# Vanlightly/vsr-tlaplus

Hardware: NVIDIA H100
Metric: unique states explored/sec (VSR.tla, shipped VSR.cfg constants) (higher is better)
Workload: dtype u32

## Files before the change

### vsr-tlaplus_b200/csrc/vsr_gpu.cu

```cuda
#include <stddef.h>
#include <stdio.h>
#include <stdlib.h>
#include <string.h>

#include <algorithm>
#include <chrono>
#include <string>
#include <vector>

#include "vsr_engine.h"

namespace vsr {

const GpuOps* find_gpu_ops(int R, int V, int K) {
#define X(r, v, k) \
    if (R == r && V == v && K == k) return GpuThunks<Layout<r, v, k>>::get();
    VSR_FOR_EACH_CONFIG(X)
#undef X
    return nullptr;
}

}

using namespace vsr;
// ... 247 lines not shown

int vsr_engine_expand(VsrEngine* e) { return vsr_engine_step(e, 0, e->n_cur, 0, nullptr, nullptr); }

int vsr_engine_insert_records(VsrEngine* e, const void* dev_records, uint64_t n) {
    if (!e->level_open) {
        int rc = engine_reset_level(e);
        if (rc) return rc;
    }
    if (n == 0) return 0;
    InsertParams q;
    fill_params(e, q.e);
    q.recs = (const uint8_t*)dev_records;
    q.n = n;
    CK(cudaEventRecord(e->ev0, e->stream));
    CK(e->g->launch_insert(q, e->stream));
    CK(cudaEventRecord(e->ev1, e->stream));
    e->st.kernel_launches++;
    CK(cudaEventSynchronize(e->ev1));
    float ms = 0;
    cudaEventElapsedTime(&ms, e->ev0, e->ev1);
    e->level_ms_acc += ms;
    e->level_ms_insert_acc += ms;
    return 0;
}

int vsr_engine_finish_level(VsrEngine* e, VsrLevelInfo* out) {
    DevCounters c;
    CK(cudaMemcpyAsync(&c, e->ctr, sizeof c, cudaMemcpyDeviceToHost, e->stream));
    e->st.bytes_d2h += sizeof c;
    CK(cudaStreamSynchronize(e->stream));
    const uint64_t fcap_total = e->frontier_cap + e->frontier_host_cap;
    if (c.tie_count > 0 && c.tie_count <= e->tie_cap && !c.overflow && c.out_count <= fcap_total) {
        const size_t tb = (size_t)e->g->tie_bytes;
        std::vector<uint8_t> host(c.tie_count * tb);
        CK(cudaMemcpyAsync(host.data(), e->ties, host.size(), cudaMemcpyDeviceToHost, e->stream));
        CK(cudaStreamSynchronize(e->stream));
        std::vector<const uint8_t*> recs;
        for (uint64_t i = 0; i < c.tie_count; i++) recs.push_back(host.data() + i * tb);
        auto key = [](const uint8_t* r) { return (const TieRec*)r; };
        std::sort(recs.begin(), recs.end(), [&](const uint8_t* a, const uint8_t* b) {
            const TieRec *x = key(a), *y = key(b);
            if (x->fp != y->fp) return x->fp < y->fp;
            if (x->check != y->check) return x->check < y->check;
            if (x->auxkey != y->auxkey) return x->auxkey < y->auxkey;
            if (x->parent != y->parent) return x->parent < y->parent;
            return x->cand < y->cand;
        });
        std::vector<uint8_t> best;
        uint64_t nbest = 0;
        for (size_t i = 0; i < recs.size(); i++) {
            if (i && key(recs[i])->fp == key(recs[i - 1])->fp && key(recs[i])->check == key(recs[i - 1])->check) continue;
            best.insert(best.end(), recs[i], recs[i] + tb);
            nbest++;
        }
        CK(cudaMemcpyAsync(e->ties, best.data(), best.size(), cudaMemcpyHostToDevice, e->stream));
        static const unsigned long long ones = ~0ull;
        CK(cudaMemcpyAsync(&e->ctr->viol_id, &ones, 8, cudaMemcpyHostToDevice, e->stream));
        CK(cudaMemsetAsync(&e->ctr->viol_which, 0, sizeof(int), e->stream));
        ExpandParams p;
        fill_params(e, p);
        CK(e->g->launch_patch(p, e->ties, nbest, c.out_count, e->stream));
        e->st.kernel_launches++;
        CK(cudaMemcpyAsync(&c, e->ctr, sizeof c, cudaMemcpyDeviceToHost, e->stream));
        CK(cudaStreamSynchronize(e->stream));
        e->st.bytes_d2h += host.size() + sizeof c;
        e->st.bytes_h2d += best.size();
    }
    VsrLevelInfo li;
    memset(&li, 0, sizeof li);
    li.new_states = c.out_count;
    li.generated = c.generated;
    li.frontier_in = e->n_cur;
    li.ties = c.ties;
    li.collisions = c.collisions;
    li.violation = c.viol_id != ~0ull;
    li.violation_id = c.viol_id;
    li.violation_mask = c.viol_which;
    li.deadlock = c.dead_id != ~0ull;
    li.deadlock_id = c.dead_id;
    li.error_code = c.error;
    li.overflow = c.overflow;
    li.ms = e->level_ms_acc;
    li.ms_insert = e->level_ms_insert_acc;
    if (c.overflow) {
        snprintf(e->last_error, sizeof e->last_error, "capacity exceeded (%s): %llu new states this level, frontier capacity %llu",
                 c.overflow == 1 ? "frontier" : (c.overflow == 2 ? "tie list" : (c.overflow == 3 ? "send buffer" : "seen-set")), (unsigned long long)c.out_count,
                 (unsigned long long)fcap_total);
    }
    if (!li.overflow && e->st.distinct + c.out_count > e->table_cap - e->table_cap / 8) {
        li.overflow = 4;
        snprintf(e->last_error, sizeof e->last_error, "capacity exceeded (seen-set): %llu distinct states in %llu slots",
                 (unsigned long long)(e->st.distinct + c.out_count), (unsigned long long)e->table_cap);
    }
    const uint64_t n_new = c.out_count <= fcap_total ? c.out_count : fcap_total;
    e->st.generated += c.generated;
    e->st.distinct += n_new;
    e->st.h2_ties += c.ties;
    e->st.fp_collisions += c.collisions;
    e->st.probe_total += c.probes;
    e->st.seconds_kernels += e->level_ms_acc * 1e-3;
    if (c.error && !e->st.error_code) e->st.error_code = c.error;
    const int gen_level = e->level + 1;
    if (e->level >= 1 && e->level - 1 < VSR_MAX_LEVELS) {
        e->st.level_generated[e->level - 1] = c.generated;
        e->st.level_ms[e->level - 1] = e->level_ms_acc;
        e->st.levels_expanded = e->level;
    }
    if (n_new > 0 && gen_level - 1 < VSR_MAX_LEVELS) {
        e->st.level_sizes[gen_level - 1] = n_new;
        e->st.num_levels = gen_level;
    }
    if (li.violation && e->st.violation_level == 0) {
        e->st.violation_level = gen_level;
        e->st.violation_id = c.viol_id;
    }
    e->cur ^= 1;
    e->cur_base = e->next_base;
    e->n_cur = n_new;
    e->next_base += n_new;
    e->level = gen_level;
    e->level_open = false;
    if (e->opts.collect_levels) {
        std::vector<uint8_t> host((size_t)n_new * e->g->bytes);
        if (n_new && vsr_engine_read_frontier(e, 0, n_new, host.data())) return VSR_RC_SYSTEM;
        e->collected.push_back(std::move(host));
    }
    if (out) *out = li;
    return 0;
}

uint64_t vsr_engine_frontier_size(const VsrEngine* e) { return e->n_cur; }

int vsr_engine_read_frontier(VsrEngine* e, uint64_t first, uint64_t n, void* host_out) {
    if (first + n > e->n_cur) return VSR_RC_ERROR;
    const uint64_t S = (uint64_t)e->g->bytes;
    const uint64_t in_dev = first < e->frontier_cap ? std::min(n, e->frontier_cap - first) : 0;
    if (in_dev) CK(cudaMemcpy(host_out, (const uint8_t*)e->frontier[e->cur] + first * S, in_dev * S, cudaMemcpyDeviceToHost));
    if (n > in_dev) memcpy((uint8_t*)host_out + in_dev * S, (const uint8_t*)e->frontier_host[e->cur] + (first + in_dev - e->frontier_cap) * S, (n - in_dev) * S);
    return 0;
}

int vsr_engine_trace_record(VsrEngine* e, uint64_t local_id, uint64_t* parent_out, uint32_t* cand_out) {
    if (!e->trace || local_id >= e->trace_cap) return VSR_RC_ERROR;
    uint64_t t = 0;
    CK(cudaMemcpy(&t, e->trace + local_id, 8, cudaMemcpyDeviceToHost));
    e->st.bytes_d2h += 8;
    *parent_out = (t >> 12) & GID_MASK;
    *cand_out = (uint32_t)(t & 0xFFF);
    return 0;
}

int vsr_engine_lookup(VsrEngine* e, const void* state, int* level_out, int* owner_out) {
    const ModelOps* ops = e->m->ops;
    uint64_t fp = ops->fingerprint((const uint32_t*)state, e->m->run.use_view);
    if (fp == 0) fp = 1;
    const int owner = e->world > 1 ? owner_of(fp, e->owner_shift) : e->rank;
    if (owner_out) *owner_out = owner;
    *level_out = 0;
    if (owner != e->rank) return 0;
    const uint32_t chk = e->g->check_hash((const uint32_t*)state, e->m->run.use_view);
    unsigned long long* d = (unsigned long long*)&e->ctr->work_next;
    lookup_kernel<<<1, 1, 0, e->stream>>>(e->table, e->table_cap, fp, chk, d);
    CK(cudaGetLastError());
    unsigned long long meta = 0;
    CK(cudaMemcpyAsync(&meta, d, 8, cudaMemcpyDeviceToHost, e->stream));
    CK(cudaStreamSynchronize(e->stream));
// ... 237 lines not shown
```

### vsr-tlaplus_b200/csrc/vsr_gpu.cuh

```cuda
#ifndef VSR_GPU_CUH
#define VSR_GPU_CUH

#include <cuda_runtime.h>
#include <stdint.h>

#include "vsr_actions.h"

namespace vsr {

struct DevCounters {
    unsigned long long out_count;
    unsigned long long generated;
    unsigned long long ties;
    unsigned long long collisions;
    unsigned long long probes;
    unsigned long long viol_id;
    unsigned long long dead_id;
    unsigned long long tie_count;
    int error;
    int overflow;
    int viol_which;
    int _pad;
    unsigned long long work_next;
    unsigned long long drain_next;
    unsigned int send_count[8];
};

struct TieRec {
    uint64_t fp;
    uint64_t parent;
    uint32_t auxkey, cand, check, _pad;
};

struct RecHdr {
    uint64_t fp;
    uint64_t tm;
};
constexpr int MAX_WORLD = 8;


struct ExpandParams {
    const uint32_t* in;
    unsigned long long n_in;
    unsigned long long in_base;
    const uint32_t* in_hi;
    unsigned long long in_split;
    uint32_t* out;
    uint32_t* out_hi;
    unsigned long long out_split;
    unsigned long long out_cap;
    unsigned long long out_base;
    uint64_t* table;
    unsigned long long table_cap;
    uint64_t* trace;
    unsigned long long trace_cap;
    DevCounters* ctr;
    uint8_t* ties;
    unsigned long long tie_cap;
    const uint64_t* fp_tab;
    RunCfg run;
    int level;
    int check_deadlock;
    int rank, world, owner_shift;
    uint8_t* push[MAX_WORLD];
    unsigned long long push_cap;
    int push_direct;
    const uint8_t* drain[MAX_WORLD];
    unsigned int drain_n[MAX_WORLD];
    unsigned long long drain_total;
};

struct InsertParams {
    const uint8_t* recs;
    unsigned long long n;
    ExpandParams e;
};


__device__ __forceinline__ void cas128(uint64_t* p, uint64_t s0, uint64_t s1, uint64_t& o0, uint64_t& o1) {
    asm volatile(
        "{\n\t.reg .b128 cmp, swp, old;\n\tmov.b128 cmp, {%2, %3};\n\tmov.b128 swp, {%4, %5};\n\t"
        "atom.global.relaxed.gpu.cas.b128 old, [%6], cmp, swp;\n\tmov.b128 {%0, %1}, old;\n\t}"
        : "=l"(o0), "=l"(o1)
        : "l"(0ull), "l"(0ull), "l"(s0), "l"(s1), "l"(p)
        : "memory");
}
__device__ __forceinline__ void ld128_cg(const uint64_t* p, uint64_t& a, uint64_t& b) {
    asm volatile("ld.global.cg.v2.u64 {%0, %1}, [%2];" : "=l"(a), "=l"(b) : "l"(p) : "memory");
}
__device__ __forceinline__ uint64_t mix64(uint64_t x) {
    x ^= x >> 30; x *= 0xbf58476d1ce4e5b9ULL;
    x ^= x >> 27; x *= 0x94d049bb133111ebULL;
    x ^= x >> 31;
    return x;
}
template <class L, bool USE_VIEW, class W> VSR_HD uint32_t check_hash_t(const W& w) {
    constexpr int full = L::VIEW_BITS >> 5, rem = L::VIEW_BITS & 31;
    constexpr int nw = USE_VIEW ? (full + (rem ? 1 : 0)) : L::NW;
    uint32_t h = 0x9747b28cu;
VSR_UNROLL
    for (int i = 0; i < nw; i++) {
        uint32_t k = rdw(w, i);
        if (USE_VIEW && i == full) k &= (1u << rem) - 1u;
        h ^= k;
        h = ((h << 13) | (h >> 19)) * 5u + 0xe6546b64u;
    }
    h ^= h >> 16; h *= 0x85ebca6bu; h ^= h >> 13; h *= 0xc2b2ae35u; h ^= h >> 16;
    return h;
}
// ... 8 lines not shown
__host__ __device__ __forceinline__ uint64_t make_trec(uint64_t parent_gid, uint32_t cand) { return (parent_gid << 12) | (cand & 0xFFFu); }

__device__ __forceinline__ uint64_t make_meta(int level, uint32_t auxkey, uint32_t check) {
    return ((uint64_t)(uint32_t)level << 56) | ((uint64_t)(auxkey & 0xFFFFFFu) << 32) | check;
}

#ifndef VSR_BUCKET
#define VSR_BUCKET 2
#endif
struct Probe { uint64_t e[2 * VSR_BUCKET]; };
__device__ __forceinline__ void ld256_cg(const uint64_t* p, uint64_t& a, uint64_t& b, uint64_t& c, uint64_t& d) {
    asm volatile("ld.global.cg.v2.u64 {%0, %1}, [%4];\n\tld.global.cg.v2.u64 {%2, %3}, [%4+16];"
                 : "=l"(a), "=l"(b), "=l"(c), "=l"(d) : "l"(p) : "memory");
}
__device__ __forceinline__ unsigned long long table_home(unsigned long long cap, uint64_t fp) {
    return __umul64hi(fp * 0x9E3779B97F4A7C15ULL, cap / VSR_BUCKET) * VSR_BUCKET;
}
__device__ __forceinline__ void probe_load(const uint64_t* table, unsigned long long h, Probe& p) {
#if VSR_BUCKET == 1
    ld128_cg(table + 2 * h, p.e[0], p.e[1]);
#elif VSR_BUCKET == 2
    ld128_cg(table + 2 * h, p.e[0], p.e[1]);
#elif VSR_BUCKET == 4
    ld256_cg(table + 2 * h, p.e[0], p.e[1], p.e[2], p.e[3]);
    ld256_cg(table + 2 * h + 4, p.e[4], p.e[5], p.e[6], p.e[7]);
#else
#error "VSR_BUCKET must be 1, 2 or 4"
#endif
}
__device__ __forceinline__ int table_insert_from(uint64_t* table, unsigned long long cap, unsigned long long h, Probe p, uint64_t fp, uint64_t meta,
                                                 unsigned& probes, unsigned& collisions) {
    for (unsigned tries = 0;; tries++) {
        if (tries > (1u << 16)) return INS_FULL;
        probes++;
VSR_UNROLL
        for (int j = 0; j < VSR_BUCKET; j++) {
            uint64_t e0, e1;
            if (VSR_BUCKET == 2 && j == 1) {
                ld128_cg(table + 2 * (h + 1), e0, e1);
            } else {
                e0 = p.e[2 * j];
                e1 = p.e[2 * j + 1];
            }
            if (e0 == 0) {
                cas128(table + 2 * (h + j), fp, meta, e0, e1);
                if (e0 == 0 && e1 == 0) return INS_NEW;
            }
            for (int again = 0; e1 == 0 && again < 64; again++) ld128_cg(table + 2 * (h + j), e0, e1);
            if (e0 == fp) {
                if ((uint32_t)e1 == (uint32_t)meta) {
                    const bool same_level = (e1 >> 56) == (meta >> 56);
                    const bool same_aux = ((e1 >> 32) & 0xFFFFFF) == ((meta >> 32) & 0xFFFFFF);
                    return (same_level && !same_aux) ? INS_TIE : INS_DUP;
                }
                collisions++;
            }
        }
        h += VSR_BUCKET;
        if (h >= cap) h = 0;
        probe_load(table, h, p);
    }
}
__device__ __forceinline__ int table_insert(uint64_t* table, unsigned long long cap, uint64_t fp, uint64_t meta,
                                            unsigned& probes, unsigned& collisions) {
    const unsigned long long h = table_home(cap, fp);
    Probe p;
    probe_load(table, h, p);
    return table_insert_from(table, cap, h, p, fp, meta, probes, collisions);
}

__device__ __forceinline__ void bulk_store(void* gdst, const void* ssrc, uint32_t bytes) {
    asm volatile("fence.proxy.async.shared::cta;" ::: "memory");
    const uint32_t s = (uint32_t)__cvta_generic_to_shared(ssrc);
    asm volatile("cp.async.bulk.global.shared::cta.bulk_group [%0], [%1], %2;" ::"l"(gdst), "r"(s), "r"(bytes) : "memory");
    asm volatile("cp.async.bulk.commit_group;" ::: "memory");
    asm volatile("cp.async.bulk.wait_group.read 0;" ::: "memory");
}

template <int NW> __device__ __forceinline__ uint32_t* out_state(const ExpandParams& P, unsigned long long i) {
    return i < P.out_split ? P.out + i * NW : P.out_hi + (i - P.out_split) * NW;
}


constexpr int SCAP = 64;
#ifdef VSR_QPS
constexpr int QPS = VSR_QPS;
#else
constexpr int QPS = 10;
#endif

template <class L> struct WarpStage {
    alignas(16) uint32_t stage[SCAP * L::NW + 32];
    unsigned long long tstage[SCAP];
    int sn;
};
template <class L, int WARPS> struct BlockSmemT {
    static constexpr int NS = WARPS * 32;
    static constexpr int NG = 13;
    uint64_t fp_tab[8 * 256];
    uint32_t par[NS * (L::NW + 1)];
    static constexpr int QCAP = QPS * NS;
    uint16_t pool[QCAP];
    int qcount[NG];
    int take;
    unsigned long long round_first;
    WarpStage<L> w[WARPS];
};
template <class L> struct ExpandCfg {
    static constexpr size_t SMEM_ONE = 227 * 1024 - 512, SMEM_TWO = 113 * 1024;
    static constexpr int max_grp() { int m = 0; for (int g = 0; g < Ops<L>::NGRP; g++) m = Ops<L>::grp_size(g) > m ? Ops<L>::grp_size(g) : m; return m; }
    template <int W> static constexpr int pick_one() {
        if constexpr (W < 18) return 0;
        else if constexpr (sizeof(BlockSmemT<L, W>) <= SMEM_ONE) return W;
        else return pick_one<W - 2>();
    }
    static constexpr int W2 = sizeof(BlockSmemT<L, 16>) <= SMEM_TWO ? 16 : (sizeof(BlockSmemT<L, 12>) <= SMEM_TWO ? 12 : 8);
    static constexpr int W1 = max_grp() < 64 ? pick_one<32>() : 0;
#ifdef VSR_FORCE_WARPS
    static constexpr int WARPS = VSR_FORCE_WARPS;
#else
    static constexpr int WARPS = W1 >= 2 * W2 - 4 ? W1 : W2;
#endif
    static constexpr int BLOCKS = WARPS > 16 ? 1 : 2;
    typedef BlockSmemT<L, WARPS> Smem;
};

template <class L, bool MULTI> struct Expander {
    typedef Ops<L> O_;
    typedef typename ExpandCfg<L>::Smem Smem;
    static constexpr int WARPS = ExpandCfg<L>::WARPS, NS = Smem::NS;
    const ExpandParams& P;
    Smem& B;
    WarpStage<L>& S;
    const int lane, warp, tid;
    const uint32_t* mine = nullptr;
    bool have = false;

    __device__ Expander(const ExpandParams& p, Smem& b) : P(p), B(b), S(b.w[threadIdx.x >> 5]), lane(threadIdx.x & 31), warp(threadIdx.x >> 5), tid(threadIdx.x) {}

    static __device__ __noinline__ void flush(const ExpandParams& P, WarpStage<L>& S, int lane, int n) {
        const int sn = S.sn;
        unsigned long long base = 0;
        if (lane == 0) base = atomicAdd(&P.ctr->out_count, (unsigned long long)n);
        base = __shfl_sync(0xffffffffu, base, 0);
        if (lane < n) {
            const unsigned long long t = S.tstage[lane];
            if (t >> 63) {
                atomicMin(&P.ctr->viol_id, P.out_base + base + lane);
                S.tstage[lane] = t & ~(1ull << 63);
            }
        }
        __syncwarp();
        if (base + n > P.out_cap) {
            if (lane == 0) atomicExch(&P.ctr->overflow, 1);
        } else {
            if (lane == 0) {
                if (base + n <= P.out_split) bulk_store(P.out + base * L::NW, S.stage, (uint32_t)(n * L::BYTES));
                else if (base >= P.out_split) bulk_store(P.out_hi + (base - P.out_split) * L::NW, S.stage, (uint32_t)(n * L::BYTES));
                else {
                    const int n1 = (int)(P.out_split - base);
                    bulk_store(P.out + base * L::NW, S.stage, (uint32_t)(n1 * L::BYTES));
                    bulk_store(P.out_hi, S.stage + n1 * L::NW, (uint32_t)((n - n1) * L::BYTES));
                }
            }
            if (P.trace && lane < n && P.out_base + base + lane < P.trace_cap) P.trace[P.out_base + base + lane] = S.tstage[lane];
        }
        __syncwarp();
        const int rest = sn - n;
        for (int i0 = 0; i0 < rest * L::NW; i0 += 32) {
            const int i = i0 + lane;
            uint32_t v = 0;
            if (i < rest * L::NW) v = S.stage[n * L::NW + i];
            __syncwarp();
            if (i < rest * L::NW) S.stage[i] = v;
        }
        unsigned long long t = 0;
        if (lane < rest) t = S.tstage[n + lane];
        __syncwarp();
        if (lane < rest) S.tstage[lane] = t;
        if (lane == 0) S.sn = rest;
        __syncwarp();
    }

    typedef uint32_t* Row;
    static constexpr int gcd32(int a) { int g = 32; while (a % g) g >>= 1; return g; }
    static constexpr int SKEW_P = 32 / gcd32(L::NW);
    static __device__ __forceinline__ Row scratch(WarpStage<L>& S, int lane) { return &S.stage[(32 + lane) * L::NW + lane / SKEW_P]; }

    static __device__ __forceinline__ void push_records(const ExpandParams& P, WarpStage<L>& S, int lane, const RegRow<L::NW>& v, int send_to, uint64_t fp,
                                                        uint64_t tm) {
        const unsigned senders = __ballot_sync(0xffffffffu, send_to >= 0);
        if (!senders) return;
        constexpr int RB = L::BYTES + (int)sizeof(RecHdr), RW = RB / 4;
        constexpr int CAPREC = (32 * L::BYTES) / RB;
        static_assert(CAPREC >= 16, "two passes must cover a batch");
        int off = 0, cnt = 0, rnk = 0;
        unsigned mymask = 0;
        for (int d = 0; d < P.world; d++) {
            const unsigned m = __ballot_sync(0xffffffffu, send_to == d);
            if (send_to > d) off += __popc(m);
            if (send_to == d) { mymask = m; cnt = __popc(m); rnk = __popc(m & ((1u << lane) - 1u)); }
        }
        unsigned base = 0;
        if (send_to >= 0 && rnk == 0) base = atomicAdd(&P.ctr->send_count[send_to], (unsigned)cnt);
        base = __shfl_sync(0xffffffffu, base, mymask ? __ffs(mymask) - 1 : 0);
        const bool fits = send_to >= 0 && (unsigned long long)base + (unsigned)cnt <= P.push_cap;
        if (send_to >= 0 && !fits && rnk == 0) atomicExch(&P.ctr->overflow, 3);
        if (P.push_direct) {
            if (fits) {
                uint4* d = reinterpret_cast<uint4*>(P.push[send_to] + (size_t)(base + (unsigned)rnk) * RB);
                VSR_UNROLL
                for (int q = 0; q < L::NW / 4; q++) d[q] = make_uint4(v.w[4 * q], v.w[4 * q + 1], v.w[4 * q + 2], v.w[4 * q + 3]);
                d[L::NW / 4] = make_uint4((uint32_t)fp, (uint32_t)(fp >> 32), (uint32_t)tm, (uint32_t)(tm >> 32));
            }
            return;
        }
        const int pos = off + rnk, total = __popc(senders);
        uint32_t* sbuf = &S.stage[32 * L::NW];
        for (int lo = 0; lo < total; lo += CAPREC) {
            const int hi = lo + CAPREC < total ? lo + CAPREC : total;
            if (send_to >= 0 && pos >= lo && pos < hi) {
                uint32_t* r = sbuf + (pos - lo) * RW;
                VSR_UNROLL
                for (int j = 0; j < L::NW; j++) r[j] = v.w[j];
                r[L::NW] = (uint32_t)fp; r[L::NW + 1] = (uint32_t)(fp >> 32);
                r[L::NW + 2] = (uint32_t)tm; r[L::NW + 3] = (uint32_t)(tm >> 32);
            }
            __syncwarp();
            if (fits) {
                const int st = off > lo ? off : lo, en = off + cnt < hi ? off + cnt : hi;
                if (pos == st && st < en)
                    bulk_store(P.push[send_to] + (size_t)(base + (unsigned)(st - off)) * RB, sbuf + (st - lo) * RW, (uint32_t)((en - st) * RB));
            }
            __syncwarp();
        }
    }

    static __device__ __forceinline__ unsigned long long commit(const ExpandParams& P, WarpStage<L>& S, int lane, const RegRow<L::NW>& v, bool live, uint64_t fp,
                                                                uint32_t chk, uint32_t auxkey, unsigned long long home, const Probe& first, unsigned long long trec,
                                                                unsigned mult, bool check_inv = true) {
        unsigned gen = 0, probes = 0, coll = 0;
        int sn = S.sn;
        bool isnew = false;
        int bad = 0;
        if (live) {
            const uint64_t meta = make_meta(P.level, auxkey, chk);
            gen = mult;
            const int r = table_insert_from(P.table, P.table_cap, home, first, fp, meta, probes, coll);
            isnew = r == INS_NEW;
            if (r == INS_FULL) atomicExch(&P.ctr->overflow, 4);
            if (isnew && check_inv) bad = O_::invariant(P.run, v);
            if (coll) atomicAdd(&P.ctr->collisions, (unsigned long long)coll);
            if (r == INS_TIE) {
                atomicAdd(&P.ctr->ties, 1ull);
                const unsigned long long t = atomicAdd(&P.ctr->tie_count, 1ull);
                if (t < P.tie_cap) {
                    TieRec rec;
                    rec.fp = fp; rec.parent = trec >> 12; rec.auxkey = auxkey; rec.cand = (uint32_t)(trec & 0xFFFu); rec.check = chk; rec._pad = 0;
                    uint8_t* dst = P.ties + t * (sizeof(TieRec) + L::BYTES);
                    *(TieRec*)dst = rec;
                    VSR_UNROLL
                    for (int j = 0; j < L::NW; j++) ((uint32_t*)(dst + sizeof(TieRec)))[j] = v.w[j];
                } else atomicExch(&P.ctr->overflow, 2);
            }
        }
        const unsigned newmask = __ballot_sync(0xffffffffu, isnew);
        __syncwarp();
        if (isnew) {
            const int slot = sn + __popc(newmask & ((1u << lane) - 1u));
            VSR_UNROLL
            for (int j = 0; j < L::NW; j++) S.stage[slot * L::NW + j] = v.w[j];
            if (bad) {
                trec |= 1ull << 63;
                atomicOr(&P.ctr->viol_which, bad);
            }
            S.tstage[slot] = trec;
        }
        sn += __popc(newmask);
        __syncwarp();
        if (lane == 0) S.sn = sn;
        __syncwarp();
        while (sn >= 32) {
            flush(P, S, lane, 32);
            sn -= 32;
        }
        return (unsigned long long)gen | ((unsigned long long)probes << 32);
    }

    static __device__ __noinline__ unsigned long long emit(const ExpandParams& P, Smem& B, WarpStage<L>& S, int lane, const Row n, int mult,
                                                           int cand, int si, bool act, bool check_inv) {
        int send_to = -1;
        uint64_t fp = 0;
        uint32_t chk = 0, auxkey = 0;
        unsigned long long home = 0, trec = 0;
        Probe first = {};
        bool live = false;
        RegRow<L::NW> v;
        if (act && mult > 0) {
            VSR_UNROLL
            for (int j = 0; j < L::NW; j++) v.w[j] = rdw(n, j);
        }
        if (act) {
            if (mult < 0) {
                atomicCAS(&P.ctr->error, 0, mult);
            } else if (mult > 0) {
                fp = fp64_view8<L>(B.fp_tab, v, P.run.use_view != 0);
                if (fp == 0) fp = 1;
                const int owner = MULTI ? owner_of(fp, P.owner_shift) : P.rank;
                trec = make_trec(make_gid(P.rank, P.in_base + B.round_first + si), (uint32_t)cand);
                if (owner == P.rank) {
                    live = true;
                    home = table_home(P.table_cap, fp);
                    probe_load(P.table, home, first);
                    chk = check_hash<L>(v, P.run.use_view != 0);
                    auxkey = O_::aux_key(v);
                } else {
                    send_to = owner;
                }
            }
        }
        if (MULTI) {
            __syncwarp();
            push_records(P, S, lane, v, send_to, fp, trec | ((uint64_t)(unsigned)mult << 56));
        }
        return commit(P, S, lane, v, live, fp, chk, auxkey, home, first, trec, (unsigned)mult, check_inv);
    }

    struct DrainPre {
        uint64_t fp, tm;
        unsigned long long home;
        Probe first;
        const uint4* rec;
        bool have;
    };
    unsigned long long dchunk = ~0ull;
    __device__ __forceinline__ unsigned long long drain_chunks() const { return (P.drain_total + 31) / 32; }
    __device__ __forceinline__ unsigned long long drain_claim() {
        unsigned long long c = 0;
        if (lane == 0) c = atomicAdd(&P.ctr->drain_next, 1ull);
        return c;
    }
    __device__ __forceinline__ DrainPre drain_begin(unsigned long long chunk) {
        constexpr int RB = L::BYTES + (int)sizeof(RecHdr);
        DrainPre d;
        unsigned long long i = chunk * 32 + lane;
        d.have = chunk < drain_chunks() && i < P.drain_total;
        d.fp = d.tm = 0;
        d.home = 0;
        d.first = Probe{};
        d.rec = nullptr;
        if (d.have) {
            int s = 0;
            while (s < P.world - 1 && i >= P.drain_n[s]) { i -= P.drain_n[s]; s++; }
            d.rec = reinterpret_cast<const uint4*>(P.drain[s] + i * RB);
            const uint4 h = __ldcs(d.rec + L::NW / 4);
            d.fp = ((uint64_t)h.y << 32) | h.x;
            d.tm = ((uint64_t)h.w << 32) | h.z;
            d.home = table_home(P.table_cap, d.fp);
            probe_load(P.table, d.home, d.first);
        }
        return d;
    }
    __device__ __forceinline__ void drain_end(const DrainPre& d) {
        RegRow<L::NW> v;
        uint32_t chk = 0, auxkey = 0;
        if (d.have) {
            VSR_UNROLL
            for (int q = 0; q < L::NW / 4; q++) {
                const uint4 x = __ldcs(d.rec + q);
                v.w[4 * q] = x.x; v.w[4 * q + 1] = x.y; v.w[4 * q + 2] = x.z; v.w[4 * q + 3] = x.w;
            }
            chk = check_hash<L>(v, P.run.use_view != 0);
            auxkey = O_::aux_key(v);
        }
        tally(commit(P, S, lane, v, d.have, d.fp, chk, auxkey, d.home, d.first, d.tm & ((1ull << 56) - 1ull), (unsigned)((d.tm >> 56) & 0xFu)));
    }
    __device__ void drain() {
        const unsigned long long nchunks = drain_chunks();
        if (dchunk == ~0ull) dchunk = __shfl_sync(0xffffffffu, drain_claim(), 0);
        while (dchunk < nchunks) {
            const unsigned long long nx = drain_claim();
            const DrainPre d = drain_begin(dchunk);
            drain_end(d);
            dchunk = __shfl_sync(0xffffffffu, nx, 0);
        }
    }

    static constexpr int NG = O_::NGRP;
    static __host__ __device__ constexpr int moff(int g) { int o = 0; for (int h = 0; h < g; h++) o += O_::grp_words(h); return o; }
    static constexpr int MW = moff(NG);
    static constexpr int PW = (NG + 1) / 2;
    static __host__ __device__ constexpr int max_grp() { int m = 0; for (int g = 0; g < NG; g++) m = O_::grp_size(g) > m ? O_::grp_size(g) : m; return m; }
    static constexpr int TBITS = NS <= 512 ? 9 : 10;
    static_assert(NS <= (1 << TBITS) && max_grp() < (1 << (16 - TBITS)), "pool item does not fit 16 bits");
    static_assert(max_grp() * NS < 65536, "16-bit packed counters");

    template <int G> __device__ __forceinline__ void guards(const RegRow<L::NW>& st, uint32_t* m, uint32_t* pc) {
        O_::template enabled_group<G>(P.run, st, m + moff(G));
        uint32_t c = 0;
        VSR_UNROLL
        for (int k = 0; k < O_::grp_words(G); k++) c += (uint32_t)__popc(m[moff(G) + k]);
        pc[G >> 1] += c << (16 * (G & 1));
        if constexpr (G + 1 < NG) guards<G + 1>(st, m, pc);
    }
    template <int G, bool FAST> __device__ __forceinline__ void push(uint32_t* m, const uint32_t* ex, const uint32_t* wb, int st) {
        int pos = st + (int)((wb[G >> 1] >> (16 * (G & 1))) & 0xFFFFu) + (int)((ex[G >> 1] >> (16 * (G & 1))) & 0xFFFFu);
        VSR_UNROLL
        for (int k = 0; k < O_::grp_words(G); k++) {
            uint32_t mm = m[moff(G) + k], left = 0;
            while (mm) {
                const int bit = __ffs(mm) - 1;
                mm &= mm - 1;
                if (FAST || pos < Smem::QCAP) B.pool[pos] = (uint16_t)(tid | ((k * 32 + bit) << TBITS));
                else left |= 1u << bit;
                pos++;
            }
            if (!FAST) m[moff(G) + k] = left;
        }
        if constexpr (G + 1 < NG) {
            const int nst = FAST ? st + B.qcount[G] : (st + B.qcount[G] < Smem::QCAP ? st + B.qcount[G] : Smem::QCAP);
            push<G + 1, FAST>(m, ex, wb, nst);
        }
    }
    template <int G> __device__ __forceinline__ void leftovers(uint32_t* m) {
        VSR_UNROLL
        for (int k = 0; k < O_::grp_words(G); k++) {
            while (__any_sync(0xffffffffu, m[moff(G) + k] != 0)) {
                const bool inl = m[moff(G) + k] != 0;
                int cand = 0;
                if (inl) {
                    const int bit = __ffs(m[moff(G) + k]) - 1;
                    m[moff(G) + k] &= m[moff(G) + k] - 1;
                    cand = O_::grp_begin(G) + k * 32 + bit;
                }
                tally(apply<G>(P, B, S, lane, mine, cand, tid, inl));
            }
        }
        if constexpr (G + 1 < NG) leftovers<G + 1>(m);
    }
    __device__ __forceinline__ void scan_all() {
        uint32_t m[MW], pc[PW];
        VSR_UNROLL
        for (int i = 0; i < MW; i++) m[i] = 0;
        VSR_UNROLL
        for (int i = 0; i < PW; i++) pc[i] = 0;
        if (have) {
            RegRow<L::NW> st;
            VSR_UNROLL
            for (int i = 0; i < L::NW; i++) st.w[i] = mine[i];
            guards<0>(st, m, pc);
        }
        uint32_t ex[PW], wb[PW];
        VSR_UNROLL
        for (int i = 0; i < PW; i++) ex[i] = pc[i];
        VSR_UNROLL
        for (int o = 1; o < 32; o <<= 1) {
            VSR_UNROLL
            for (int i = 0; i < PW; i++) {
                const uint32_t t = __shfl_up_sync(0xffffffffu, ex[i], o);
                if (lane >= o) ex[i] += t;
            }
        }
        uint32_t mytot = 0, anyc = 0;
        VSR_UNROLL
        for (int g = 0; g < NG; g++) {
            const uint32_t t = (__shfl_sync(0xffffffffu, ex[g >> 1], 31) >> (16 * (g & 1))) & 0xFFFFu;
            if (lane == g) mytot = t;
        }
        VSR_UNROLL
        for (int i = 0; i < PW; i++) { anyc |= pc[i]; ex[i] -= pc[i]; }
        uint32_t mybase = 0;
        if (lane < NG && mytot) mybase = (uint32_t)atomicAdd(&B.qcount[lane], (int)mytot);
        VSR_UNROLL
        for (int i = 0; i < PW; i++) wb[i] = 0;
        VSR_UNROLL
        for (int g = 0; g < NG; g++) wb[g >> 1] |= (__shfl_sync(0xffffffffu, mybase, g) & 0xFFFFu) << (16 * (g & 1));
        if (P.check_deadlock && have && !anyc) atomicMin(&P.ctr->dead_id, P.in_base + B.round_first + tid);
        __syncthreads();
#ifndef VSR_EXP_NO_PUSHFAST
        int all = 0;
        VSR_UNROLL
        for (int g = 0; g < NG; g++) all += B.qcount[g];
        if (all <= Smem::QCAP) {
            push<0, true>(m, ex, wb, 0);
            return;
        }
#endif
        push<0, false>(m, ex, wb, 0);
        uint32_t rest = 0;
        VSR_UNROLL
        for (int i = 0; i < MW; i++) rest |= m[i];
        if (__any_sync(0xffffffffu, rest != 0)) leftovers<0>(m);
    }
    template <int G> static __device__ __noinline__ unsigned long long apply(const ExpandParams& P, Smem& B, WarpStage<L>& S, int lane,
                                                                             const uint32_t* parent, int cand, int si, bool act) {
        const Row n = scratch(S, lane);
        int mult = 0;
        if (act) mult = O_::template step_grp<true, G>(P.run, parent, cand, n);
#ifdef VSR_EXP_INVSKIP
        return emit(P, B, S, lane, n, mult, cand, si, act, O_::may_falsify(G));
#else
        return emit(P, B, S, lane, n, mult, cand, si, act, true);
#endif
    }
    template <int G> static __device__ __forceinline__ unsigned long long batch(const ExpandParams& P, Smem& B, WarpStage<L>& S, int lane, int b,
                                                                                int k) {
        const bool act = lane < k;
        int cand = 0, si = 0;
        if (act) {
            const unsigned item = B.pool[b + lane];
            si = item & ((1 << TBITS) - 1);
            cand = O_::grp_begin(G) + (int)(item >> TBITS);
        }
        return apply<G>(P, B, S, lane, &B.par[si * (L::NW + 1)], cand, si, act);
    }
    unsigned long long acc_gen = 0, acc_probes = 0;
    __device__ __forceinline__ void tally(unsigned long long r) {
        acc_gen += (unsigned)r;
        acc_probes += r >> 32;
    }

    __device__ void run_round(unsigned long long first, int count) {
        const uint32_t* src = P.in + first * L::NW;
        if (first + count <= P.in_split) {
            for (int i = tid; i < count * L::NW; i += NS) B.par[(i / L::NW) * (L::NW + 1) + (i % L::NW)] = __ldg(src + i);
        } else {
            for (int i = tid; i < count * L::NW; i += NS) {
                const unsigned long long st = first + i / L::NW;
                const uint32_t* row = st < P.in_split ? P.in + st * L::NW : P.in_hi + (st - P.in_split) * L::NW;
                B.par[(i / L::NW) * (L::NW + 1) + (i % L::NW)] = __ldg(row + i % L::NW);
            }
        }
        if (tid < Smem::NG) B.qcount[tid] = 0;
        if (tid == 0) { B.round_first = first; B.take = 0; }
        __syncthreads();
        have = tid < count;
        mine = &B.par[(have ? tid : 0) * (L::NW + 1)];
        scan_all();
        __syncthreads();
        const int q = lane < Smem::NG ? B.qcount[lane] : 0;
        int inc = q;
        VSR_UNROLL
        for (int o = 1; o < 32; o <<= 1) {
            const int t = __shfl_up_sync(0xffffffffu, inc, o);
            if (lane >= o) inc += t;
        }
        const int seg_st = inc - q < Smem::QCAP ? inc - q : Smem::QCAP, seg_en = inc < Smem::QCAP ? inc : Smem::QCAP;
        const int nb = (seg_en - seg_st + 31) >> 5;
        int binc = nb;
        VSR_UNROLL
        for (int o = 1; o < 32; o <<= 1) {
            const int t = __shfl_up_sync(0xffffffffu, binc, o);
            if (lane >= o) binc += t;
        }
        const int total = __shfl_sync(0xffffffffu, binc, 31);
        for (;;) {
            int t = 0;
            if (lane == 0) t = atomicAdd(&B.take, 1);
            t = __shfl_sync(0xffffffffu, t, 0);
            if (t >= total) break;
            const int g = __popc(__ballot_sync(0xffffffffu, lane < Smem::NG && binc <= t));
            const int st = __shfl_sync(0xffffffffu, seg_st, g), en = __shfl_sync(0xffffffffu, seg_en, g);
            const int b = st + (t - __shfl_sync(0xffffffffu, binc - nb, g)) * 32;
            const int k = en - b < 32 ? en - b : 32;
            unsigned long long r;
            switch (g) {
            case 0: r = batch<0>(P, B, S, lane, b, k); break;   case 1: r = batch<1>(P, B, S, lane, b, k); break;
            case 2: r = batch<2>(P, B, S, lane, b, k); break;   case 3: r = batch<3>(P, B, S, lane, b, k); break;
            case 4: r = batch<4>(P, B, S, lane, b, k); break;   case 5: r = batch<5>(P, B, S, lane, b, k); break;
            case 6: r = batch<6>(P, B, S, lane, b, k); break;   case 7: r = batch<7>(P, B, S, lane, b, k); break;
            case 8: r = batch<8>(P, B, S, lane, b, k); break;   case 9: r = batch<9>(P, B, S, lane, b, k); break;
            case 10: r = batch<10>(P, B, S, lane, b, k); break; case 11: r = batch<11>(P, B, S, lane, b, k); break;
            default: r = batch<12>(P, B, S, lane, b, k); break;
            }
            tally(r);
        }
    }

    __device__ void finish() {
        while (S.sn > 0) flush(P, S, lane, S.sn < 32 ? S.sn : 32);
        for (int o = 16; o; o >>= 1) {
            acc_gen += __shfl_xor_sync(0xffffffffu, acc_gen, o);
            acc_probes += __shfl_xor_sync(0xffffffffu, acc_probes, o);
        }
        if (lane == 0) {
            atomicAdd(&P.ctr->generated, acc_gen);
            atomicAdd(&P.ctr->probes, acc_probes);
        }
    }
};

template <class L, bool MULTI> __global__ void __launch_bounds__(ExpandCfg<L>::WARPS * 32, ExpandCfg<L>::BLOCKS) expand_kernel(const __grid_constant__ ExpandParams P) {
    extern __shared__ __align__(128) unsigned char smem_raw[];
    typedef typename ExpandCfg<L>::Smem Smem;
    Smem& B = *reinterpret_cast<Smem*>(smem_raw);
    for (int i = threadIdx.x; i < 8 * 256; i += blockDim.x) B.fp_tab[i] = P.fp_tab[i];
    __shared__ unsigned long long next_round;
    Expander<L, MULTI> X(P, B);
    if ((threadIdx.x & 31) == 0) {
        WarpStage<L>& S = B.w[threadIdx.x >> 5];
        S.sn = 0;
    }
    const unsigned long long nrounds = (P.n_in + Smem::NS - 1) / Smem::NS;
    if (threadIdx.x == 0) next_round = atomicAdd(&P.ctr->work_next, 1ull);
    for (;;) {
        __syncthreads();
        const unsigned long long c = next_round;
        __syncthreads();
        if (c >= nrounds) break;
        if (threadIdx.x == 0) {
            next_round = atomicAdd(&P.ctr->work_next, 1ull);
            const unsigned long long nx = next_round;
            if (nx < nrounds && (nx + 1) * Smem::NS <= P.in_split) {
                const unsigned long long nfirst = nx * Smem::NS;
                const unsigned long long ncount = (P.n_in - nfirst) < (unsigned long long)Smem::NS ? (P.n_in - nfirst) : Smem::NS;
                asm volatile("cp.async.bulk.prefetch.L2.global [%0], %1;" ::"l"(P.in + nfirst * L::NW), "r"((uint32_t)(ncount * L::BYTES)) : "memory");
            }
        }
        const unsigned long long first = c * Smem::NS;
        const int count = (int)((P.n_in - first) < (unsigned long long)Smem::NS ? (P.n_in - first) : Smem::NS);
        X.run_round(first, count);
    }
    if (MULTI && P.drain_total) X.drain();
    X.finish();
}


template <class L> __global__ void __launch_bounds__(256) insert_kernel(const InsertParams Q) {
    const ExpandParams& P = Q.e;
    const unsigned long long i = (unsigned long long)blockIdx.x * blockDim.x + threadIdx.x;
    const int lane = threadIdx.x & 31;
    const bool have = i < Q.n;
    bool isnew = false;
    const uint8_t* rec = Q.recs + (have ? i : 0) * (L::BYTES + sizeof(RecHdr));
    const uint32_t* n = (const uint32_t*)rec;
    const RecHdr* h = (const RecHdr*)(rec + L::BYTES);
    unsigned probes = 0, coll = 0, nties = 0;
    unsigned long long gen = 0;
    uint64_t parent = 0;
    uint32_t cand = 0;
    if (have) {
        const uint64_t meta = make_meta(P.level, Ops<L>::aux_key(n), check_hash<L>(n, P.run.use_view != 0));
        const int r = table_insert(P.table, P.table_cap, h->fp, meta, probes, coll);
        isnew = r == INS_NEW;
        if (r == INS_FULL) atomicExch(&P.ctr->overflow, 4);
        gen = (h->tm >> 56) & 0xFu;
        parent = (h->tm >> 12) & ((1ull << 44) - 1ull);
        cand = (uint32_t)(h->tm & 0xFFFu);
        if (r == INS_TIE) {
            nties = 1;
            const unsigned long long t = atomicAdd(&P.ctr->tie_count, 1ull);
            if (t < P.tie_cap) {
                TieRec tr;
                tr.fp = h->fp; tr.parent = parent; tr.auxkey = (uint32_t)((meta >> 32) & 0xFFFFFF); tr.cand = cand;
                tr.check = (uint32_t)meta; tr._pad = 0;
                uint8_t* dst = P.ties + t * (sizeof(TieRec) + L::BYTES);
                *(TieRec*)dst = tr;
                for (int j = 0; j < L::NW; j++) ((uint32_t*)(dst + sizeof(TieRec)))[j] = n[j];
            } else atomicExch(&P.ctr->overflow, 2);
        }
    }
    for (int o = 16; o; o >>= 1) {
        gen += __shfl_xor_sync(0xffffffffu, gen, o);
        probes += __shfl_xor_sync(0xffffffffu, probes, o);
        coll += __shfl_xor_sync(0xffffffffu, coll, o);
        nties += __shfl_xor_sync(0xffffffffu, nties, o);
    }
    if (lane == 0) {
        if (gen) atomicAdd(&P.ctr->generated, gen);
        if (probes) atomicAdd(&P.ctr->probes, (unsigned long long)probes);
        if (coll) atomicAdd(&P.ctr->collisions, (unsigned long long)coll);
        if (nties) atomicAdd(&P.ctr->ties, (unsigned long long)nties);
    }
    const unsigned newmask = __ballot_sync(0xffffffffu, isnew);
    if (newmask) {
        unsigned long long base = 0;
        const int leader = __ffs(newmask) - 1;
        if (lane == leader) base = atomicAdd(&P.ctr->out_count, (unsigned long long)__popc(newmask));
        base = __shfl_sync(0xffffffffu, base, leader);
        if (isnew) {
            const unsigned long long pos = base + __popc(newmask & ((1u << lane) - 1u));
            if (pos < P.out_cap) {
                uint32_t* dst = out_state<L::NW>(P, pos);
                for (int j = 0; j < L::NW; j++) dst[j] = n[j];
                if (P.trace && P.out_base + pos < P.trace_cap) P.trace[P.out_base + pos] = make_trec(parent, cand);
                const int bad = Ops<L>::invariant(P.run, n);
                if (bad) {
                    atomicMin(&P.ctr->viol_id, P.out_base + pos);
                    atomicOr(&P.ctr->viol_which, bad);
                }
            } else atomicExch(&P.ctr->overflow, 1);
        }
    }
}

template <class L> __global__ void patch_ties_kernel(const ExpandParams P, const uint8_t* ties, unsigned long long ntie, unsigned long long n_out) {
    const unsigned long long i = (unsigned long long)blockIdx.x * blockDim.x + threadIdx.x;
    if (i >= n_out) return;
    uint32_t w[L::NW];
    uint32_t* st = out_state<L::NW>(P, i);
    for (int j = 0; j < L::NW; j++) w[j] = st[j];
    uint64_t fp = fp64_view8<L>(P.fp_tab, w, P.run.use_view != 0);
    if (fp == 0) fp = 1;
// ... 105 lines not shown
```

Before: 2.658 billion.

## Scan two frontier passes per round to halve block barriers per state

Each block round now covers PASSES×NS parent states. The scan phase runs once per pass, into separate queue-count and pool segments, and then a single batch phase drains both passes' candidate queues, amortising the round-end and scan barriers over twice the states. To fit in shared memory, the per-warp staging buffer shrinks to 32 rows when two passes are used, so commit flushes immediately instead of accumulating up to 64 rows. This means more global atomics on out_count and smaller bulk stores. Optional clock64 instrumentation behind a macro breaks round time into barrier, scan and batch components.

Result: faster. 2.963 billion (median of 6 runs) (+11.5%).

```diff
diff --git a/vsr-tlaplus_b200/csrc/vsr_gpu.cu b/vsr-tlaplus_b200/csrc/vsr_gpu.cu
--- a/vsr-tlaplus_b200/csrc/vsr_gpu.cu
+++ b/vsr-tlaplus_b200/csrc/vsr_gpu.cu
@@ -353,6 +353,15 @@
     li.overflow = c.overflow;
     li.ms = e->level_ms_acc;
     li.ms_insert = e->level_ms_insert_acc;
+#ifdef VSR_EXP_ROUNDCLK
+    {
+        double all = 0;
+        for (int i = 0; i < 5; i++) all += (double)c.roundclk[i];
+        if (all > 0)
+            fprintf(stderr, "roundclk rank %d depth %d  ms %.4f  warp-Gcycles %.4f  end_barrier %.4f  scan_barriers %.4f  batches %.4f  scan %.4f  other %.4f\n",
+                    e->rank, e->level, e->level_ms_acc, all * 1e-9, c.roundclk[0] / all, c.roundclk[1] / all, c.roundclk[2] / all, c.roundclk[3] / all, c.roundclk[4] / all);
+    }
+#endif
     if (c.overflow) {
         snprintf(e->last_error, sizeof e->last_error, "capacity exceeded (%s): %llu new states this level, frontier capacity %llu",
                  c.overflow == 1 ? "frontier" : (c.overflow == 2 ? "tie list" : (c.overflow == 3 ? "send buffer" : "seen-set")), (unsigned long long)c.out_count,
diff --git a/vsr-tlaplus_b200/csrc/vsr_gpu.cuh b/vsr-tlaplus_b200/csrc/vsr_gpu.cuh
--- a/vsr-tlaplus_b200/csrc/vsr_gpu.cuh
+++ b/vsr-tlaplus_b200/csrc/vsr_gpu.cuh
@@ -24,7 +24,13 @@
     unsigned long long work_next;
     unsigned long long drain_next;
     unsigned int send_count[8];
+#ifdef VSR_EXP_ROUNDCLK
+    unsigned long long roundclk[5];
+#endif
 };
+#ifdef VSR_EXP_ROUNDCLK
+enum { CLK_END = 0, CLK_SCANBAR = 1, CLK_BATCH = 2, CLK_SCAN = 3, CLK_OTHER = 4 };
+#endif
 
 struct TieRec {
     uint64_t fp;
@@ -199,39 +205,40 @@
 }
 
 
-constexpr int SCAP = 64;
 #ifdef VSR_QPS
 constexpr int QPS = VSR_QPS;
 #else
 constexpr int QPS = 10;
 #endif
 
-template <class L> struct WarpStage {
-    alignas(16) uint32_t stage[SCAP * L::NW + 32];
-    unsigned long long tstage[SCAP];
+template <class L, int ROWS> struct WarpStage {
+    alignas(16) uint32_t stage[ROWS * L::NW + 32];
+    unsigned long long tstage[ROWS];
     int sn;
 };
-template <class L, int WARPS> struct BlockSmemT {
+template <class L, int WARPS, int PASSES> struct BlockSmemT {
+    typedef WarpStage<L, PASSES == 2 ? 32 : 64> Stage;
     static constexpr int NS = WARPS * 32;
+    static constexpr int NR = PASSES * NS;
     static constexpr int NG = 13;
     uint64_t fp_tab[8 * 256];
-    uint32_t par[NS * (L::NW + 1)];
+    uint32_t par[NR * (L::NW + 1)];
     static constexpr int QCAP = QPS * NS;
-    uint16_t pool[QCAP];
-    int qcount[NG];
+    uint16_t pool[PASSES * QCAP];
+    int qcount[PASSES][NG];
     int take;
     unsigned long long round_first;
-    WarpStage<L> w[WARPS];
+    Stage w[WARPS];
 };
 template <class L> struct ExpandCfg {
     static constexpr size_t SMEM_ONE = 227 * 1024 - 512, SMEM_TWO = 113 * 1024;
     static constexpr int max_grp() { int m = 0; for (int g = 0; g < Ops<L>::NGRP; g++) m = Ops<L>::grp_size(g) > m ? Ops<L>::grp_size(g) : m; return m; }
     template <int W> static constexpr int pick_one() {
         if constexpr (W < 18) return 0;
-        else if constexpr (sizeof(BlockSmemT<L, W>) <= SMEM_ONE) return W;
+        else if constexpr (sizeof(BlockSmemT<L, W, 1>) <= SMEM_ONE) return W;
         else return pick_one<W - 2>();
     }
-    static constexpr int W2 = sizeof(BlockSmemT<L, 16>) <= SMEM_TWO ? 16 : (sizeof(BlockSmemT<L, 12>) <= SMEM_TWO ? 12 : 8);
+    static constexpr int W2 = sizeof(BlockSmemT<L, 16, 1>) <= SMEM_TWO ? 16 : (sizeof(BlockSmemT<L, 12, 1>) <= SMEM_TWO ? 12 : 8);
     static constexpr int W1 = max_grp() < 64 ? pick_one<32>() : 0;
 #ifdef VSR_FORCE_WARPS
     static constexpr int WARPS = VSR_FORCE_WARPS;
@@ -239,24 +246,49 @@
     static constexpr int WARPS = W1 >= 2 * W2 - 4 ? W1 : W2;
 #endif
     static constexpr int BLOCKS = WARPS > 16 ? 1 : 2;
-    typedef BlockSmemT<L, WARPS> Smem;
+#ifdef VSR_ROUND_PASSES
+    static constexpr int PASSES = VSR_ROUND_PASSES;
+#else
+    static constexpr int PASSES = BLOCKS == 1 && sizeof(BlockSmemT<L, WARPS, 2>) <= SMEM_ONE ? 2 : 1;
+#endif
+    typedef BlockSmemT<L, WARPS, PASSES> Smem;
 };
 
 template <class L, bool MULTI> struct Expander {
     typedef Ops<L> O_;
     typedef typename ExpandCfg<L>::Smem Smem;
-    static constexpr int WARPS = ExpandCfg<L>::WARPS, NS = Smem::NS;
+    typedef typename Smem::Stage Stage;
+    static constexpr int WARPS = ExpandCfg<L>::WARPS, NS = Smem::NS, PASSES = ExpandCfg<L>::PASSES;
+    static constexpr int SROWS = PASSES == 2 ? 32 : 64;
     const ExpandParams& P;
     Smem& B;
-    WarpStage<L>& S;
+    Stage& S;
     const int lane, warp, tid;
     const uint32_t* mine = nullptr;
     bool have = false;
-
-    __device__ Expander(const ExpandParams& p, Smem& b) : P(p), B(b), S(b.w[threadIdx.x >> 5]), lane(threadIdx.x & 31), warp(threadIdx.x >> 5), tid(threadIdx.x) {}
-
-    static __device__ __noinline__ void flush(const ExpandParams& P, WarpStage<L>& S, int lane, int n) {
-        const int sn = S.sn;
+    int pass = 0;
+    __device__ __forceinline__ int pass_i() const { return PASSES == 1 ? 0 : pass; }
+
+    __device__ Expander(const ExpandParams& p, Smem& b) : P(p), B(b), S(b.w[threadIdx.x >> 5]), lane(threadIdx.x & 31), warp(threadIdx.x >> 5), tid(threadIdx.x) {
+#ifdef VSR_EXP_ROUNDCLK
+        clk_t = clock64();
+#endif
+    }
+
+#ifdef VSR_EXP_ROUNDCLK
+    unsigned long long clk_t = 0, clk[5] = {};
+    __device__ __forceinline__ void clk_mark(int i) {
+        const unsigned long long t = clock64();
+        clk[i] += t - clk_t;
+        clk_t = t;
+    }
+#define VSR_CLK(X, i) (X).clk_mark(CLK_##i)
+#else
+#define VSR_CLK(X, i) ((void)0)
+#endif
+
+    static __device__ __noinline__ void flush(const ExpandParams& P, Stage& S, int lane, int n) {
+        const int sn = SROWS == 32 ? n : S.sn;
         unsigned long long base = 0;
         if (lane == 0) base = atomicAdd(&P.ctr->out_count, (unsigned long long)n);
         base = __shfl_sync(0xffffffffu, base, 0);
@@ -302,9 +334,9 @@
     typedef uint32_t* Row;
     static constexpr int gcd32(int a) { int g = 32; while (a % g) g >>= 1; return g; }
     static constexpr int SKEW_P = 32 / gcd32(L::NW);
-    static __device__ __forceinline__ Row scratch(WarpStage<L>& S, int lane) { return &S.stage[(32 + lane) * L::NW + lane / SKEW_P]; }
-
-    static __device__ __forceinline__ void push_records(const ExpandParams& P, WarpStage<L>& S, int lane, const RegRow<L::NW>& v, int send_to, uint64_t fp,
+    static __device__ __forceinline__ Row scratch(Stage& S, int lane) { return &S.stage[(SROWS - 32 + lane) * L::NW + lane / SKEW_P]; }
+
+    static __device__ __forceinline__ void push_records(const ExpandParams& P, Stage& S, int lane, const RegRow<L::NW>& v, int send_to, uint64_t fp,
                                                         uint64_t tm) {
         const unsigned senders = __ballot_sync(0xffffffffu, send_to >= 0);
         if (!senders) return;
@@ -333,7 +365,7 @@
             return;
         }
         const int pos = off + rnk, total = __popc(senders);
-        uint32_t* sbuf = &S.stage[32 * L::NW];
+        uint32_t* sbuf = &S.stage[(SROWS - 32) * L::NW];
         for (int lo = 0; lo < total; lo += CAPREC) {
             const int hi = lo + CAPREC < total ? lo + CAPREC : total;
             if (send_to >= 0 && pos >= lo && pos < hi) {
@@ -353,11 +385,11 @@
         }
     }
 
-    static __device__ __forceinline__ unsigned long long commit(const ExpandParams& P, WarpStage<L>& S, int lane, const RegRow<L::NW>& v, bool live, uint64_t fp,
+    static __device__ __forceinline__ unsigned long long commit(const ExpandParams& P, Stage& S, int lane, const RegRow<L::NW>& v, bool live, uint64_t fp,
                                                                 uint32_t chk, uint32_t auxkey, unsigned long long home, const Probe& first, unsigned long long trec,
                                                                 unsigned mult, bool check_inv = true) {
         unsigned gen = 0, probes = 0, coll = 0;
-        int sn = S.sn;
+        int sn = SROWS == 32 ? 0 : S.sn;
         bool isnew = false;
         int bad = 0;
         if (live) {
@@ -395,16 +427,20 @@
         }
         sn += __popc(newmask);
         __syncwarp();
-        if (lane == 0) S.sn = sn;
-        __syncwarp();
-        while (sn >= 32) {
-            flush(P, S, lane, 32);
-            sn -= 32;
+        if constexpr (SROWS == 32) {
+            if (newmask) flush(P, S, lane, sn);
+        } else {
+            if (lane == 0) S.sn = sn;
+            __syncwarp();
+            while (sn >= 32) {
+                flush(P, S, lane, 32);
+                sn -= 32;
+            }
         }
         return (unsigned long long)gen | ((unsigned long long)probes << 32);
     }
 
-    static __device__ __noinline__ unsigned long long emit(const ExpandParams& P, Smem& B, WarpStage<L>& S, int lane, const Row n, int mult,
+    static __device__ __noinline__ unsigned long long emit(const ExpandParams& P, Smem& B, Stage& S, int lane, const Row n, int mult,
                                                            int cand, int si, bool act, bool check_inv) {
         int send_to = -1;
         uint64_t fp = 0;
@@ -528,14 +564,15 @@
             while (mm) {
                 const int bit = __ffs(mm) - 1;
                 mm &= mm - 1;
-                if (FAST || pos < Smem::QCAP) B.pool[pos] = (uint16_t)(tid | ((k * 32 + bit) << TBITS));
+                if (FAST || pos < Smem::QCAP) B.pool[pass_i() * Smem::QCAP + pos] = (uint16_t)(tid | ((k * 32 + bit) << TBITS));
                 else left |= 1u << bit;
                 pos++;
             }
             if (!FAST) m[moff(G) + k] = left;
         }
         if constexpr (G + 1 < NG) {
-            const int nst = FAST ? st + B.qcount[G] : (st + B.qcount[G] < Smem::QCAP ? st + B.qcount[G] : Smem::QCAP);
+            const int q = B.qcount[pass_i()][G];
+            const int nst = FAST ? st + q : (st + q < Smem::QCAP ? st + q : Smem::QCAP);
             push<G + 1, FAST>(m, ex, wb, nst);
         }
     }
@@ -550,7 +587,7 @@
                     m[moff(G) + k] &= m[moff(G) + k] - 1;
                     cand = O_::grp_begin(G) + k * 32 + bit;
                 }
-                tally(apply<G>(P, B, S, lane, mine, cand, tid, inl));
+                tally(apply<G>(P, B, S, lane, mine, cand, pass_i() * NS + tid, inl));
             }
         }
         if constexpr (G + 1 < NG) leftovers<G + 1>(m);
@@ -587,17 +624,19 @@
         VSR_UNROLL
         for (int i = 0; i < PW; i++) { anyc |= pc[i]; ex[i] -= pc[i]; }
         uint32_t mybase = 0;
-        if (lane < NG && mytot) mybase = (uint32_t)atomicAdd(&B.qcount[lane], (int)mytot);
+        if (lane < NG && mytot) mybase = (uint32_t)atomicAdd(&B.qcount[pass_i()][lane], (int)mytot);
         VSR_UNROLL
         for (int i = 0; i < PW; i++) wb[i] = 0;
         VSR_UNROLL
         for (int g = 0; g < NG; g++) wb[g >> 1] |= (__shfl_sync(0xffffffffu, mybase, g) & 0xFFFFu) << (16 * (g & 1));
-        if (P.check_deadlock && have && !anyc) atomicMin(&P.ctr->dead_id, P.in_base + B.round_first + tid);
+        if (P.check_deadlock && have && !anyc) atomicMin(&P.ctr->dead_id, P.in_base + B.round_first + pass_i() * NS + tid);
+        VSR_CLK(*this, SCAN);
         __syncthreads();
+        VSR_CLK(*this, SCANBAR);
 #ifndef VSR_EXP_NO_PUSHFAST
         int all = 0;
         VSR_UNROLL
-        for (int g = 0; g < NG; g++) all += B.qcount[g];
+        for (int g = 0; g < NG; g++) all += B.qcount[pass_i()][g];
         if (all <= Smem::QCAP) {
             push<0, true>(m, ex, wb, 0);
             return;
@@ -609,7 +648,7 @@
         for (int i = 0; i < MW; i++) rest |= m[i];
         if (__any_sync(0xffffffffu, rest != 0)) leftovers<0>(m);
     }
-    template <int G> static __device__ __noinline__ unsigned long long apply(const ExpandParams& P, Smem& B, WarpStage<L>& S, int lane,
+    template <int G> static __device__ __noinline__ unsigned long long apply(const ExpandParams& P, Smem& B, Stage& S, int lane,
                                                                              const uint32_t* parent, int cand, int si, bool act) {
         const Row n = scratch(S, lane);
         int mult = 0;
@@ -620,13 +659,13 @@
         return emit(P, B, S, lane, n, mult, cand, si, act, true);
 #endif
     }
-    template <int G> static __device__ __forceinline__ unsigned long long batch(const ExpandParams& P, Smem& B, WarpStage<L>& S, int lane, int b,
+    template <int G> static __device__ __forceinline__ unsigned long long batch(const ExpandParams& P, Smem& B, Stage& S, int lane, int b,
                                                                                 int k) {
         const bool act = lane < k;
         int cand = 0, si = 0;
         if (act) {
             const unsigned item = B.pool[b + lane];
-            si = item & ((1 << TBITS) - 1);
+            si = (PASSES == 1 ? 0 : b / Smem::QCAP) * NS + (int)(item & ((1 << TBITS) - 1));
             cand = O_::grp_begin(G) + (int)(item >> TBITS);
         }
         return apply<G>(P, B, S, lane, &B.par[si * (L::NW + 1)], cand, si, act);
@@ -648,21 +687,32 @@
                 B.par[(i / L::NW) * (L::NW + 1) + (i % L::NW)] = __ldg(row + i % L::NW);
             }
         }
-        if (tid < Smem::NG) B.qcount[tid] = 0;
+        if (tid < PASSES * Smem::NG) (&B.qcount[0][0])[tid] = 0;
         if (tid == 0) { B.round_first = first; B.take = 0; }
+        VSR_CLK(*this, SCAN);
         __syncthreads();
-        have = tid < count;
-        mine = &B.par[(have ? tid : 0) * (L::NW + 1)];
-        scan_all();
+        VSR_CLK(*this, SCANBAR);
+#pragma unroll 1
+        for (pass = 0; pass < PASSES; pass++) {
+            have = pass_i() * NS + tid < count;
+            mine = &B.par[(have ? pass_i() * NS + tid : 0) * (L::NW + 1)];
+            scan_all();
+        }
+        VSR_CLK(*this, SCAN);
         __syncthreads();
-        const int q = lane < Smem::NG ? B.qcount[lane] : 0;
+        VSR_CLK(*this, SCANBAR);
+        static_assert(PASSES * Smem::NG <= 32, "one lane per segment");
+        const int sp = lane / Smem::NG;
+        const int q = lane < PASSES * Smem::NG ? (&B.qcount[0][0])[lane] : 0;
         int inc = q;
         VSR_UNROLL
         for (int o = 1; o < 32; o <<= 1) {
             const int t = __shfl_up_sync(0xffffffffu, inc, o);
             if (lane >= o) inc += t;
         }
-        const int seg_st = inc - q < Smem::QCAP ? inc - q : Smem::QCAP, seg_en = inc < Smem::QCAP ? inc : Smem::QCAP;
+        const int before = __shfl_sync(0xffffffffu, inc, sp * Smem::NG - 1 + (sp == 0));
+        if (sp > 0) inc -= before;
+        const int seg_st = sp * Smem::QCAP + (inc - q < Smem::QCAP ? inc - q : Smem::QCAP), seg_en = sp * Smem::QCAP + (inc < Smem::QCAP ? inc : Smem::QCAP);
         const int nb = (seg_en - seg_st + 31) >> 5;
         int binc = nb;
         VSR_UNROLL
@@ -676,12 +726,12 @@
             if (lane == 0) t = atomicAdd(&B.take, 1);
             t = __shfl_sync(0xffffffffu, t, 0);
             if (t >= total) break;
-            const int g = __popc(__ballot_sync(0xffffffffu, lane < Smem::NG && binc <= t));
-            const int st = __shfl_sync(0xffffffffu, seg_st, g), en = __shfl_sync(0xffffffffu, seg_en, g);
-            const int b = st + (t - __shfl_sync(0xffffffffu, binc - nb, g)) * 32;
+            const int s = __popc(__ballot_sync(0xffffffffu, lane < PASSES * Smem::NG && binc <= t));
+            const int st = __shfl_sync(0xffffffffu, seg_st, s), en = __shfl_sync(0xffffffffu, seg_en, s);
+            const int b = st + (t - __shfl_sync(0xffffffffu, binc - nb, s)) * 32;
             const int k = en - b < 32 ? en - b : 32;
             unsigned long long r;
-            switch (g) {
+            switch (s % Smem::NG) {
             case 0: r = batch<0>(P, B, S, lane, b, k); break;   case 1: r = batch<1>(P, B, S, lane, b, k); break;
             case 2: r = batch<2>(P, B, S, lane, b, k); break;   case 3: r = batch<3>(P, B, S, lane, b, k); break;
             case 4: r = batch<4>(P, B, S, lane, b, k); break;   case 5: r = batch<5>(P, B, S, lane, b, k); break;
@@ -691,11 +741,19 @@
             default: r = batch<12>(P, B, S, lane, b, k); break;
             }
             tally(r);
-        }
+            VSR_CLK(*this, BATCH);
+        }
+        VSR_CLK(*this, BATCH);
     }
 
     __device__ void finish() {
         while (S.sn > 0) flush(P, S, lane, S.sn < 32 ? S.sn : 32);
+#ifdef VSR_EXP_ROUNDCLK
+        clk_mark(CLK_OTHER);
+        VSR_UNROLL
+        for (int i = 0; i < 5; i++)
+            if (lane == 0) atomicAdd(&P.ctr->roundclk[i], clk[i]);
+#endif
         for (int o = 16; o; o >>= 1) {
             acc_gen += __shfl_xor_sync(0xffffffffu, acc_gen, o);
             acc_probes += __shfl_xor_sync(0xffffffffu, acc_probes, o);
@@ -714,28 +772,27 @@
     for (int i = threadIdx.x; i < 8 * 256; i += blockDim.x) B.fp_tab[i] = P.fp_tab[i];
     __shared__ unsigned long long next_round;
     Expander<L, MULTI> X(P, B);
-    if ((threadIdx.x & 31) == 0) {
-        WarpStage<L>& S = B.w[threadIdx.x >> 5];
-        S.sn = 0;
-    }
-    const unsigned long long nrounds = (P.n_in + Smem::NS - 1) / Smem::NS;
+    if ((threadIdx.x & 31) == 0) B.w[threadIdx.x >> 5].sn = 0;
+    const unsigned long long nrounds = (P.n_in + Smem::NR - 1) / Smem::NR;
     if (threadIdx.x == 0) next_round = atomicAdd(&P.ctr->work_next, 1ull);
+    VSR_CLK(X, OTHER);
     for (;;) {
         __syncthreads();
         const unsigned long long c = next_round;
         __syncthreads();
+        VSR_CLK(X, END);
         if (c >= nrounds) break;
         if (threadIdx.x == 0) {
             next_round = atomicAdd(&P.ctr->work_next, 1ull);
             const unsigned long long nx = next_round;
-            if (nx < nrounds && (nx + 1) * Smem::NS <= P.in_split) {
-                const unsigned long long nfirst = nx * Smem::NS;
-                const unsigned long long ncount = (P.n_in - nfirst) < (unsigned long long)Smem::NS ? (P.n_in - nfirst) : Smem::NS;
+            if (nx < nrounds && (nx + 1) * Smem::NR <= P.in_split) {
+                const unsigned long long nfirst = nx * Smem::NR;
+                const unsigned long long ncount = (P.n_in - nfirst) < (unsigned long long)Smem::NR ? (P.n_in - nfirst) : Smem::NR;
                 asm volatile("cp.async.bulk.prefetch.L2.global [%0], %1;" ::"l"(P.in + nfirst * L::NW), "r"((uint32_t)(ncount * L::BYTES)) : "memory");
             }
         }
-        const unsigned long long first = c * Smem::NS;
-        const int count = (int)((P.n_in - first) < (unsigned long long)Smem::NS ? (P.n_in - first) : Smem::NS);
+        const unsigned long long first = c * Smem::NR;
+        const int count = (int)((P.n_in - first) < (unsigned long long)Smem::NR ? (P.n_in - first) : Smem::NR);
         X.run_round(first, count);
     }
     if (MULTI && P.drain_total) X.drain();
```
